# KristinnVikarJ/nbody-simulation

Hardware: AMD Instinct MI355X
Metric: pair-interactions/sec + ms/step at N=1M direct O(N^2) (force + integration step) (higher is better)
Workload: dtype f32; 1 GPU; direct O(N^2) f32, N=1048576 bodies, seeded 2-D Plummer sphere, masses 1, dt=0.1, clamp=0.001 (BASELINE.json configs[2]); n_bodies=1048576, targets_per_gpu=1048576, n_ranks=1, entry=one process per GPU (sharding.py over nbody_direct_{prep,run}_dev), exchange=none, arith=AUTO (FAST kernel; EXACT on hazardous positions)

## Files before the change

nbody-simulation_amd/csrc/ctx.h:

```cpp
#pragma once
#include <hip/hip_runtime.h>

#include <cstdlib>
#include <string>
#include <tuple>
#include <vector>

#include "common.h"
#include "env.h"
#include "tree_build.hpp"

namespace nbody {

struct Multi;

template <class T> struct State {
  using T2 = typename Vec2T<T>::type;
  struct Set {
    T2* pos = nullptr;
    T2* vel = nullptr;
    uint32_t* weight = nullptr;
    uint32_t* ids = nullptr;
    T* mass = nullptr;
  };
  int64_t n = 0;
  Set set[2];
  int cur = 0;
  T2* pos_next = nullptr;
  float uniform_mass = 0.f;
  float sparse_base = 0.f;
  struct MassClasses {
    uint64_t epoch = ~0ull;
    bool usable = false;
    int n_classes = 0;
    int64_t n_slots = 0;
    int n_pad_slots = 0;
    uint32_t* rank = nullptr;
    uint32_t* pad_slots = nullptr;
    float* tile_mass = nullptr;
  } classes;
  uint64_t row_epoch = 0;
  T2* acc = nullptr;
  void* geom0 = nullptr;
  void* geom1 = nullptr;
  void* link = nullptr;
  size_t node_cap = 0;
  uint32_t* order_dev = nullptr;
  TreeHost<T> tree;
  bool tree_valid = false;
  bool tree_host_stale = false;
  int n_nodes = 0, tree_kind = 0, tree_max_depth = 0;
  int shard_kind = 0;
  int* node_depth = nullptr;
  uint32_t* node_mass = nullptr;
  T2* node_size = nullptr;
  size_t node_aux_cap = 0;
  char* qb_scratch = nullptr;
  size_t qb_scratch_bytes = 0;
  char* bb_scratch = nullptr;
  size_t bb_scratch_bytes = 0;
  bool h_weight_stale = false;
  int quad_depth_hint = 0;
  int bvh_levels_hint = 0;
  int bvh_levels_stable = 0;
  bool bb_flags_clean = false;
  bool ahead_total_due = false;
  char* ws_scratch = nullptr;
  size_t ws_scratch_bytes = 0;
  void* ws_terms = nullptr;
  int64_t ws_capacity = 0;
  int ws_backoff = 0;
  int64_t wt_hist_n = -1, wt_hist_begin = 0;
  unsigned long long wt_total = 0;
  uint32_t* wt_hist = nullptr;
  std::vector<T> h_pos;
  std::vector<uint32_t> h_weight;
  std::vector<uint32_t> h_tmp;
};


struct Tracers {
  int64_t m = 0;
  void* pos = nullptr;
  void* vel = nullptr;
  void* acc = nullptr;
  uint8_t* mark = nullptr;
};

struct DeltaStream {
  void* keys[3] = {nullptr, nullptr, nullptr};
  int cur = 0;
  uint8_t* widths = nullptr;
  uint32_t *words = nullptr, *offsets = nullptr;
  void* scan = nullptr;
  size_t scan_bytes = 0;
  uint64_t *payload = nullptr, *total = nullptr, *htotal = nullptr;
  uint8_t* host = nullptr;
  int64_t n = -1;
  int bits = 0;
  bool key_next = true, pending = false;
  size_t stream_bytes = 0;
  uint64_t step = 0;
};

template <class T> inline float direct_mass_hint(const State<T>& s) { return s.uniform_mass > 0.f ? s.uniform_mass : -s.sparse_base; }

struct DirectStep {
  hipStream_t stream = nullptr;
  int64_t n_src = 0;
  const void *pos_all = nullptr, *mass_all = nullptr;
  float uniform_mass = 0.f, clamp = 0.f;
  int arith = 0;
  int64_t n_tgt_total = 0, n_tgt_max = 0;
  void* ws = nullptr;
  size_t ws_bytes = 0;
};
struct DirectBlock {
  int64_t tgt_begin = 0, n_tgt = 0;
  void *vel = nullptr, *pos_out = nullptr, *acc_out = nullptr;
  float delta = 0.f;
  nbody_timer* timer = nullptr;
};

struct DirectGraphKey {
  int64_t n = -1;
  const void *pos_a = nullptr, *pos_b = nullptr, *vel = nullptr, *mass = nullptr, *ws = nullptr;
  float delta = 0.f, clamp = 0.f, uniform = 0.f;
  int arith = -1;
  uint64_t row_epoch = ~0ull;
  bool cls_usable = false;
  const void *cls_rank = nullptr, *cls_tile_mass = nullptr;
  std::string env;
  auto tied() const { return std::tie(n, pos_a, pos_b, vel, mass, ws, delta, clamp, uniform, arith, row_epoch, cls_usable, cls_rank, cls_tile_mass, env); }
  bool operator==(const DirectGraphKey& o) const { return tied() == o.tied(); }
};
struct DirectGraph {
  hipGraphExec_t exec = nullptr;
  DirectGraphKey key;
  void reset() {
    if (exec) (void)hipGraphExecDestroy(exec);
    exec = nullptr;
    key = DirectGraphKey{};
  }
};
inline std::string direct_env_signature() {
  std::string sig;
  const char* nf = getenv("NBODY_DIRECT_NEARFAR");
  sig += nf ? nf : "-";
  sig += ';';
  for (const char* k : {"NBODY_DIRECT_ASM", "NBODY_DIRECT_TPT", "NBODY_DIRECT_GSPLIT", "NBODY_DIRECT_NO_UNIFORM", "NBODY_DIRECT_NO_CLASSES",
                        "NBODY_DIRECT_NO_SPARSE",
                        "NBODY_DIRECT_MUTUAL_MIN_N"}) {
    const char* v = lab_str(k);
    sig += v ? v : "-";
    sig += ';';
  }
  return sig;
}

struct PhaseEvents {
  hipEvent_t e[4] = {nullptr, nullptr, nullptr, nullptr};
  bool borrowed = false;
};
struct PhaseTiming {
  unsigned long long* stamp_dev = nullptr;
  std::vector<int> stamp_pending;
  int stamp_next = 0;
  int stamp_open = -1;
  std::vector<PhaseEvents> pending;
  std::vector<hipEvent_t> free_events;
  nbody_counting* counter = nullptr;
  void release() {
    if (stamp_dev) (void)hipFree(stamp_dev);
    for (auto& p : pending)
      for (int k = p.borrowed ? 1 : 0; k < 4; ++k)
        if (p.e[k]) (void)hipEventDestroy(p.e[k]);
    for (auto e : free_events) (void)hipEventDestroy(e);
  }
};
struct StepAheadRecord {
  int verdict[2];
  int build[128];
  int info_before[8];
  int info_after[8];
};
static_assert(sizeof(StepAheadRecord) == (2 + 128 + 8 + 8) * sizeof(int), "the record's parts lie back to back");
constexpr int kAheadBuildWords = sizeof(StepAheadRecord::build) / sizeof(int);
}

struct nbody_ctx {
  nbody::Multi* multi = nullptr;
  int64_t row_capacity = 0;
  nbody::DirectGraph direct_graph;
  int device = 0;
  hipStream_t stream = nullptr;
  std::string err;
  nbody_params params{};
  nbody_counting counting{};
  nbody_timer* timer = nullptr;
  bool has_f32 = false, has_f64 = false;
  nbody::State<float> sf;
  nbody::State<double> sd;
  void* workspace = nullptr;
  int bvh_stops = 0;
  bool last_build_device = false;
  size_t workspace_bytes = 0;
  unsigned long long* stats_dev = nullptr;
  uint32_t* frame_work = nullptr;
  hipStream_t copy_stream = nullptr;
  hipEvent_t snap_event = nullptr;
  bool snap_pending = false;
  uint64_t steps_done = 0, snap_step = 0;
  void *snap_pos = nullptr, *snap_vel = nullptr, *snap_hpos = nullptr, *snap_hvel = nullptr;
  uint32_t *snap_w = nullptr, *snap_ids = nullptr, *snap_hw = nullptr, *snap_hids = nullptr;
  size_t snap_bytes2 = 0;
  int64_t snap_n = 0;
  bool snap_f64 = false;
  void *snap_tpos = nullptr, *snap_tvel = nullptr, *snap_htpos = nullptr, *snap_htvel = nullptr;
  size_t snap_tcap = 0;
  int64_t snap_m = 0;
  nbody::DeltaStream dl;
  nbody::DeltaStream tdl;
  uint8_t* frame_rgba = nullptr;
  uint32_t frame_px = 0;
  unsigned long long last_stats[3] = {0, 0, 0};
  bool want_stats = false;
  nbody::PhaseTiming phases;
  int* spec_dev = nullptr;
  nbody::StepAheadRecord* spec_host_dev = nullptr;
  nbody::StepAheadRecord* spec_host = nullptr;
  hipEvent_t spec_event = nullptr;
  void* probe_ws = nullptr;
  size_t probe_ws_bytes = 0;
  nbody::Tracers tracers;
};

namespace nbody {
int ctx_fail(nbody_ctx* c, int code, const std::string& msg);
int ctx_create_single(nbody_ctx** out, int device_id);
void ctx_destroy_single(nbody_ctx* c);
int ctx_upload(nbody_ctx* c, bool f64, int64_t n, const void* pos, const void* vel, const uint32_t* w);
int ctx_update_tree(nbody_ctx* c, bool f64, int kind, double delta, int n_steps, nbody_counting* counter);
int ctx_update_tree_shard(nbody_ctx* c, bool f64, int kind, double delta, int64_t begin, int64_t count, nbody_counting* counter);
int ctx_export_slice(nbody_ctx* c, int64_t begin, int64_t count, void* rows, void* pos, void* vel);
int ctx_import_rows(nbody_ctx* c, int64_t n_rows, const void* rows, const void* pos, const void* vel);
size_t ctx_direct_ws_bytes(int64_t n_src, int64_t n_tgt);
int ctx_ensure_workspace(nbody_ctx* c, size_t bytes);
int ctx_ensure_mass_classes(nbody_ctx* c);
int ctx_direct_prep(nbody_ctx* c, const DirectStep& step);
int ctx_direct_run(nbody_ctx* c, const DirectStep& step, const DirectBlock& block);
int ctx_accel_direct_at(nbody_ctx* c, bool f64, int64_t n_targets, const void* target_xy, void* acc_xy);
void multi_destroy(nbody_ctx* front);
int multi_set_params(nbody_ctx* front);
int multi_upload(nbody_ctx* front, bool f64, int64_t n, const void* pos, const void* vel, const uint32_t* w);
nbody_ctx* multi_peek(const nbody_ctx* front);
int multi_primary(nbody_ctx* front, nbody_ctx** out);
int multi_replicate(nbody_ctx* front);
int multi_update_direct(nbody_ctx* front, float delta, int n_steps, nbody_counting* counter);
int multi_accel_direct_at(nbody_ctx* front, bool f64, int64_t n_targets, const void* target_xy, void* acc_xy);
int multi_update_tree(nbody_ctx* front, bool f64, int kind, double delta, int n_steps, nbody_counting* counter);
}
```

nbody-simulation_amd/csrc/direct_mutual.hip:

```cpp
#include <hip/hip_runtime.h>
#include <stdint.h>

#include "direct_kernels.h"
#include "mutual_schedule.h"

namespace nbody {

namespace {

typedef float v2f __attribute__((ext_vector_type(2)));

constexpr int kWaves = 8;

constexpr int kSlice = kMutualSlice;
constexpr int kSliceCouples = kSlice / 2;
constexpr int kChunks = kSliceCouples / 64;
constexpr float kMarker = 1e30f;

__device__ __forceinline__ bool gate_open(const DirectArgs& a) { return a.run_state < 0 || a.flags[kFlagState] == a.run_state; }

__device__ __forceinline__ float4 couple_or_marker(const float4* c, int64_t k, int64_t n_couples) {
  return k < n_couples ? c[k] : make_float4(kMarker, kMarker, kMarker, kMarker);
}

#define NB_PX(K, H, D) "v_pk_add_f32 v[" D "], v[184:185], %[tx" #K "] op_sel:[0," #H "] op_sel_hi:[1," #H "] neg_lo:[0,1] neg_hi:[0,1]\n\t"
#define NB_PY(K, H, D) "v_pk_add_f32 v[" D "], v[186:187], %[ty" #K "] op_sel:[0," #H "] op_sel_hi:[1," #H "] neg_lo:[0,1] neg_hi:[0,1]\n\t"
#define NB_SQ(DX, DY, Q) "v_pk_mul_f32 v[" Q "], v[" DX "], v[" DX "]\n\tv_pk_fma_f32 v[" Q "], v[" DY "], v[" DY "], v[" Q "]\n\t"
#define NB_AD(XL, XH, YL, YH, SL, SH) "v_add_f32_e64 v" SL ", |v" XL "|, |v" YL "|\n\tv_add_f32_e64 v" SH ", |v" XH "|, |v" YH "|\n\t"
#define NB_DN(S, Q) "v_pk_fma_f32 v[" S "], v[" S "], v[" Q "], %[b]\n\t"
#define NB_RC(SL, SH) "v_rcp_f32_e32 v" SL ", v" SL "\n\tv_rcp_f32_e32 v" SH ", v" SH "\n\t"
#define NB_AC(T, DX, DY, S)                                                                                                          \
  "v_pk_fma_f32 %[ax" #T "], v[" DX "], v[" S "], %[ax" #T "]\n\t"                                                                    \
  "v_pk_fma_f32 v[188:189], v[" DX "], v[" S "], v[188:189] neg_lo:[1,0,0] neg_hi:[1,0,0]\n\t"                                                  \
  "v_pk_fma_f32 %[ay" #T "], v[" DY "], v[" S "], %[ay" #T "]\n\t"                                                                    \
  "v_pk_fma_f32 v[190:191], v[" DY "], v[" S "], v[190:191] neg_lo:[1,0,0] neg_hi:[1,0,0]\n\t"
#define NB_HALF(K0, K1, K2, K3, T0, T1, T2, T3, T4, T5, T6, T7)                                                                    \
  NB_PX(K0, 0, "192:193") NB_PX(K0, 1, "200:201") NB_PX(K1, 0, "208:209") NB_PX(K1, 1, "216:217")                                   \
  NB_PX(K2, 0, "224:225") NB_PX(K2, 1, "232:233") NB_PX(K3, 0, "240:241") NB_PX(K3, 1, "248:249")                                   \
  NB_PY(K0, 0, "194:195") NB_PY(K0, 1, "202:203") NB_PY(K1, 0, "210:211") NB_PY(K1, 1, "218:219")                                   \
  NB_PY(K2, 0, "226:227") NB_PY(K2, 1, "234:235") NB_PY(K3, 0, "242:243") NB_PY(K3, 1, "250:251")                                   \
  NB_SQ("192:193", "194:195", "196:197") NB_SQ("200:201", "202:203", "204:205") NB_SQ("208:209", "210:211", "212:213")             \
  NB_SQ("216:217", "218:219", "220:221") NB_SQ("224:225", "226:227", "228:229") NB_SQ("232:233", "234:235", "236:237")             \
  NB_SQ("240:241", "242:243", "244:245") NB_SQ("248:249", "250:251", "252:253")                                                    \
  "s_setprio 0\n\t"                                                                                                                \
  NB_AD("192", "193", "194", "195", "198", "199") NB_AD("200", "201", "202", "203", "206", "207")                                  \
  NB_AD("208", "209", "210", "211", "214", "215") NB_AD("216", "217", "218", "219", "222", "223")                                  \
  NB_AD("224", "225", "226", "227", "230", "231") NB_AD("232", "233", "234", "235", "238", "239")                                  \
  NB_AD("240", "241", "242", "243", "246", "247") NB_AD("248", "249", "250", "251", "254", "255")                                  \
  "s_setprio 1\n\t"                                                                                                                \
  NB_DN("198:199", "196:197") NB_DN("206:207", "204:205") NB_DN("214:215", "212:213") NB_DN("222:223", "220:221")                 \
  NB_DN("230:231", "228:229") NB_DN("238:239", "236:237") NB_DN("246:247", "244:245") NB_DN("254:255", "252:253")                 \
  NB_RC("198", "199")                                                                                                              \
  NB_RC("206", "207") NB_AC(T0, "192:193", "194:195", "198:199")                                                                   \
  NB_RC("214", "215") NB_AC(T1, "200:201", "202:203", "206:207")                                                                   \
  NB_RC("222", "223") NB_AC(T2, "208:209", "210:211", "214:215")                                                                   \
  NB_RC("230", "231") NB_AC(T3, "216:217", "218:219", "222:223")                                                                   \
  NB_RC("238", "239") NB_AC(T4, "224:225", "226:227", "230:231")                                                                   \
  NB_RC("246", "247") NB_AC(T5, "232:233", "234:235", "238:239")                                                                   \
  NB_RC("254", "255") NB_AC(T6, "240:241", "242:243", "246:247")                                                                   \
  NB_AC(T7, "248:249", "250:251", "254:255")
#define NB_ROT(R) "v_mov_b32_dpp " R ", " R " wave_ror:1 row_mask:0xf bank_mask:0xf\n\t"

__device__ __forceinline__ void mutual_steps(const v2f* tx, const v2f* ty, v2f* ax, v2f* ay, float4& rc, float4& sacc, int steps,
                                             unsigned long long bias2) {
  asm volatile("v_mov_b32 v184, %[r0]\n\tv_mov_b32 v185, %[r1]\n\tv_mov_b32 v186, %[r2]\n\tv_mov_b32 v187, %[r3]\n\t"
               "v_mov_b32 v188, %[o0]\n\tv_mov_b32 v189, %[o1]\n\tv_mov_b32 v190, %[o2]\n\tv_mov_b32 v191, %[o3]\n\t"
               "s_mov_b32 s88, %[n]\n"
               ".Lnb_mutual_%=:\n\t"
               NB_HALF(0, 1, 2, 3, 0, 1, 2, 3, 4, 5, 6, 7) NB_HALF(4, 5, 6, 7, 8, 9, 10, 11, 12, 13, 14, 15)
               NB_ROT("v184") NB_ROT("v185") NB_ROT("v186") NB_ROT("v187") NB_ROT("v188") NB_ROT("v189") NB_ROT("v190") NB_ROT("v191")
               "s_sub_u32 s88, s88, 1\n\t"
               "s_cmp_lg_u32 s88, 0\n\t"
               "s_cbranch_scc1 .Lnb_mutual_%=\n\t"
               "v_mov_b32 %[o0], v188\n\tv_mov_b32 %[o1], v189\n\tv_mov_b32 %[o2], v190\n\tv_mov_b32 %[o3], v191\n\t"
               "v_mov_b32 %[r0], v184\n\tv_mov_b32 %[r1], v185\n\tv_mov_b32 %[r2], v186\n\tv_mov_b32 %[r3], v187\n\t"
               : [ax0] "+v"(ax[0]), [ax1] "+v"(ax[1]), [ax2] "+v"(ax[2]), [ax3] "+v"(ax[3]), [ax4] "+v"(ax[4]), [ax5] "+v"(ax[5]),
                 [ax6] "+v"(ax[6]), [ax7] "+v"(ax[7]), [ax8] "+v"(ax[8]), [ax9] "+v"(ax[9]), [ax10] "+v"(ax[10]), [ax11] "+v"(ax[11]),
                 [ax12] "+v"(ax[12]), [ax13] "+v"(ax[13]), [ax14] "+v"(ax[14]), [ax15] "+v"(ax[15]),
                 [ay0] "+v"(ay[0]), [ay1] "+v"(ay[1]), [ay2] "+v"(ay[2]), [ay3] "+v"(ay[3]), [ay4] "+v"(ay[4]), [ay5] "+v"(ay[5]),
                 [ay6] "+v"(ay[6]), [ay7] "+v"(ay[7]), [ay8] "+v"(ay[8]), [ay9] "+v"(ay[9]), [ay10] "+v"(ay[10]), [ay11] "+v"(ay[11]),
                 [ay12] "+v"(ay[12]), [ay13] "+v"(ay[13]), [ay14] "+v"(ay[14]), [ay15] "+v"(ay[15]),
                 [o0] "+v"(sacc.x), [o1] "+v"(sacc.y), [o2] "+v"(sacc.z), [o3] "+v"(sacc.w),
                 [r0] "+v"(rc.x), [r1] "+v"(rc.y), [r2] "+v"(rc.z), [r3] "+v"(rc.w)
               : [tx0] "v"(tx[0]), [tx1] "v"(tx[1]), [tx2] "v"(tx[2]), [tx3] "v"(tx[3]), [tx4] "v"(tx[4]), [tx5] "v"(tx[5]),
                 [tx6] "v"(tx[6]), [tx7] "v"(tx[7]), [ty0] "v"(ty[0]), [ty1] "v"(ty[1]), [ty2] "v"(ty[2]), [ty3] "v"(ty[3]),
                 [ty4] "v"(ty[4]), [ty5] "v"(ty[5]), [ty6] "v"(ty[6]), [ty7] "v"(ty[7]), [b] "s"(bias2), [n] "s"(steps)
               : "v184", "v185", "v186", "v187", "v188", "v189", "v190", "v191",
                 "v192", "v193", "v194", "v195", "v196", "v197", "v198", "v199", "v200", "v201", "v202", "v203", "v204", "v205",
                 "v206", "v207", "v208", "v209", "v210", "v211", "v212", "v213", "v214", "v215", "v216", "v217", "v218", "v219",
                 "v220", "v221", "v222", "v223", "v224", "v225", "v226", "v227", "v228", "v229", "v230", "v231", "v232", "v233",
                 "v234", "v235", "v236", "v237", "v238", "v239", "v240", "v241", "v242", "v243", "v244", "v245", "v246", "v247",
                 "v248", "v249", "v250", "v251", "v252", "v253", "v254", "v255", "s88", "scc");
}
#undef NB_PX
#undef NB_PY
#undef NB_SQ
#undef NB_AD
#undef NB_DN
#undef NB_RC
#undef NB_AC
#undef NB_HALF
#undef NB_ROT

__device__ __forceinline__ void load_targets(const float4* couples, int64_t n_couples, int s, int w, int lane, v2f* tx, v2f* ty) {
  const int64_t tc0 = (int64_t)s * kSliceCouples + 512 * w + 8 * lane;
#pragma unroll
  for (int k = 0; k < 8; ++k) {
    const float4 c = couple_or_marker(couples, tc0 + k, n_couples);
    tx[k] = v2f{c.x, c.y};
    ty[k] = v2f{c.z, c.w};
  }
}

__device__ __forceinline__ void zero_acc(v2f* ax, v2f* ay) {
#pragma unroll
  for (int t = 0; t < 16; ++t) ax[t] = ay[t] = v2f{0.f, 0.f};
}

__device__ __forceinline__ void add_chunk(const v2f* ax, const v2f* ay, float* tot_x, float* tot_y) {
#pragma unroll
  for (int t = 0; t < 16; ++t) {
    tot_x[t] += ax[t].x + ax[t].y;
    tot_y[t] += ay[t].x + ay[t].y;
  }
}

constexpr unsigned long long kBias2 = 0x1280000012800000ull;

__device__ __forceinline__ void off_item(const float4* couples, int64_t n_couples, int s, int b, int w, int lane, float4 (*red)[kWaves][64],
                                         float2* tpart, float2* spart_f2) {
  v2f tx[8], ty[8];
  load_targets(couples, n_couples, s, w, lane, tx, ty);
  float tot_x[16], tot_y[16];
#pragma unroll
  for (int t = 0; t < 16; ++t) tot_x[t] = tot_y[t] = 0.f;
  float* spart = reinterpret_cast<float*>(spart_f2);
  for (int c = 0; c < kChunks; ++c) {
    float4 rc = couple_or_marker(couples, (int64_t)b * kSliceCouples + 64 * c + lane, n_couples);
    v2f ax[16], ay[16];
    zero_acc(ax, ay);
    float4 sacc = make_float4(0.f, 0.f, 0.f, 0.f);
    mutual_steps(tx, ty, ax, ay, rc, sacc, 64, kBias2);
    add_chunk(ax, ay, tot_x, tot_y);
    red[c & 1][w][lane] = sacc;
    __syncthreads();
    if (threadIdx.x < 256) {
      const int q = threadIdx.x >> 2, comp = threadIdx.x & 3;
      float r = 0.f;
#pragma unroll
      for (int v = 0; v < kWaves; ++v) r += reinterpret_cast<const float*>(&red[c & 1][v][q])[comp];
      spart[(size_t)(128 * c + 2 * q + (comp & 1)) * 2 + (comp >> 1)] = r;
    }
  }
#pragma unroll
  for (int t = 0; t < 16; ++t) tpart[1024 * w + 16 * lane + t] = make_float2(tot_x[t], tot_y[t]);
}

__device__ __forceinline__ void diag_item(const float4* couples, int64_t n_couples, int s, int w, int lane, float4 (*src)[8][64],
                                          float2* out) {
  using namespace mutual_schedule;
  v2f tx[8], ty[8];
  load_targets(couples, n_couples, s, w, lane, tx, ty);
  float tot_x[16], tot_y[16];
#pragma unroll
  for (int t = 0; t < 16; ++t) tot_x[t] = tot_y[t] = 0.f;
  const int64_t c0 = (int64_t)s * kSliceCouples;
  for (int p = 0; p < kDiagPhases; ++p) {
    const int u = diag_block(w, p), r0 = diag_first_step(w, p), n = diag_steps(p);
    for (int j = 0; j < 8; ++j) {
      float4 rc = couple_or_marker(couples, c0 + 512 * u + 8 * ((lane - r0) & 63) + j, n_couples);
      v2f ax[16], ay[16];
      zero_acc(ax, ay);
      float4 sacc = make_float4(0.f, 0.f, 0.f, 0.f);
      int moved;
      if (p == 0) {
        mutual_steps(tx, ty, ax, ay, rc, sacc, 1, kBias2);
        sacc = make_float4(0.f, 0.f, 0.f, 0.f);
        mutual_steps(tx, ty, ax, ay, rc, sacc, n - 2, kBias2);
        const float4 keep = sacc;
        mutual_steps(tx, ty, ax, ay, rc, sacc, 1, kBias2);
        sacc = keep;
        moved = n - 1;
      } else {
        mutual_steps(tx, ty, ax, ay, rc, sacc, n, kBias2);
        moved = n;
      }
      add_chunk(ax, ay, tot_x, tot_y);
      const int shift = (r0 + moved) & 63;
      if (shift) {
        const int from = (lane + shift) & 63;
        sacc = make_float4(__shfl(sacc.x, from), __shfl(sacc.y, from), __shfl(sacc.z, from), __shfl(sacc.w, from));
      }
      float4& d = src[u][j][lane];
      if (p == 0) {
        d = sacc;
      } else {
        const float4 o = d;
        d = make_float4(o.x + sacc.x, o.y + sacc.y, o.z + sacc.z, o.w + sacc.w);
      }
    }
    __syncthreads();
  }
#pragma unroll
  for (int k = 0; k < 8; ++k) {
    const float4 q = src[w][k][lane];
    out[1024 * w + 16 * lane + 2 * k] = make_float2(tot_x[2 * k] + q.x, tot_y[2 * k] + q.z);
    out[1024 * w + 16 * lane + 2 * k + 1] = make_float2(tot_x[2 * k + 1] + q.y, tot_y[2 * k + 1] + q.w);
  }
  __syncthreads();
}

__global__ __launch_bounds__(kWaves * 64) void direct_mutual(const DirectArgs a, MutualArea m, int64_t lo) {
  if (!gate_open(a)) return;
  const int nb = m.n_slices;
  int s, b;
  mutual_schedule::unit_slices(lo + blockIdx.x, nb, s, b);
  const int lane = threadIdx.x & 63;
  const int w = __builtin_amdgcn_readfirstlane((int)(threadIdx.x >> 6));
  const float4* couples = reinterpret_cast<const float4*>(a.src_pos);
  const int64_t n_couples = a.n_src / 2;
  float2* tpart = m.tpart + (size_t)blockIdx.x * kSlice;
  float2* spart = m.spart + (size_t)blockIdx.x * kSlice;
  __shared__ float4 lds[8][8][64];
  __builtin_amdgcn_s_setprio(1);
  if (s < b) {
    off_item(couples, n_couples, s, b, w, lane, reinterpret_cast<float4(*)[kWaves][64]>(&lds[0][0][0]), tpart, spart);
  } else {
    diag_item(couples, n_couples, s, w, lane, lds, tpart);
    if (s + 1 < nb) diag_item(couples, n_couples, s + 1, w, lane, lds, spart);
  }
}

__global__ __launch_bounds__(256) void direct_mutual_near(const DirectArgs a, MutualArea m) {
  if (!gate_open(a)) return;
  const int n_near = a.flags[kFlagNearCount];
  const float4* couples = reinterpret_cast<const float4*>(a.src_pos);
  const int n_couples = a.n_src / 2;
  const int per = (n_couples + kMutualNearSplit - 1) / kMutualNearSplit;
  const int q0 = blockIdx.x * per, q1 = q0 + per < n_couples ? q0 + per : n_couples;
  __shared__ float2 red[256];
  for (int k = blockIdx.y; k < n_near; k += gridDim.y) {
    const float2 p = a.pos_all[a.near_list[k]];
    float ax = 0.f, ay = 0.f;
#pragma unroll 4
    for (int q = q0 + (int)threadIdx.x; q < q1; q += 256) {
      const float4 c = couples[q];
#pragma unroll
      for (int h = 0; h < 2; ++h) {
        const float dx = (h ? c.y : c.x) - p.x, dy = (h ? c.w : c.z) - p.y;
        const float sum = __builtin_fabsf(dx) + __builtin_fabsf(dy);
        const float d2 = __builtin_fmaf(dy, dy, dx * dx);
        const float s = __builtin_amdgcn_rcpf(__builtin_fmaf(sum, d2, 8.0779356694631609e-28f));
        ax = __builtin_fmaf(dx, s, ax);
        ay = __builtin_fmaf(dy, s, ay);
      }
    }
    red[threadIdx.x] = make_float2(ax, ay);
    __syncthreads();
    for (int w = 128; w > 0; w >>= 1) {
      if ((int)threadIdx.x < w) {
        red[threadIdx.x].x += red[threadIdx.x + w].x;
        red[threadIdx.x].y += red[threadIdx.x + w].y;
      }
      __syncthreads();
    }
    if (threadIdx.x == 0) m.near_part[(size_t)k * kMutualNearSplit + blockIdx.x] = red[0];
    __syncthreads();
  }
}

__global__ __launch_bounds__(256) void direct_mutual_reduce(const DirectArgs a, MutualArea m, int64_t lo, int64_t hi, int first, int last) {
  using mutual_schedule::item_of;
  if (!gate_open(a)) return;
  const int i = blockIdx.x * 256 + threadIdx.x;
  if (i >= a.n_tgt) return;
  const int nb = m.n_slices;
  const int s = i / kSlice, l = i % kSlice;
  int r0 = 0, r1 = s;
  while (r0 < r1) {
    const int mid = (r0 + r1) >> 1;
    if (item_of(mid, s, nb) < lo) r0 = mid + 1; else r1 = mid;
  }
  int re = s;
  r1 = r0;
  while (r1 < re) {
    const int mid = (r1 + re) >> 1;
    if (item_of(mid, s, nb) < hi) r1 = mid + 1; else re = mid;
  }
  const int64_t b0 = s + 1 < nb ? item_of(s, s + 1, nb) : 0, b1 = s + 1 < nb ? item_of(s, nb - 1, nb) + 1 : 0;
  const int64_t w0 = b0 > lo ? b0 : lo, w1 = b1 < hi ? b1 : hi;
  const int64_t d = mutual_schedule::diag_unit(s, nb);
  const bool has_d = d >= lo && d < hi;
  if (r0 == r1 && w0 >= w1 && !has_d && !first && !last) return;
  float2 acc = first ? make_float2(0.f, 0.f) : a.partial[i];
#pragma unroll 8
  for (int r = r0; r < r1; ++r) {
    const float2 p = m.spart[(size_t)(item_of(r, s, nb) - lo) * kSlice + l];
    acc.x += p.x;
    acc.y += p.y;
  }
#pragma unroll 8
  for (int64_t it = w0; it < w1; ++it) {
    const float2 p = m.tpart[(size_t)(it - lo) * kSlice + l];
    acc.x += p.x;
    acc.y += p.y;
  }
  if (has_d) {
    const float2 p = ((s & 1) ? m.spart : m.tpart)[(size_t)(d - lo) * kSlice + l];
    acc.x += p.x;
    acc.y += p.y;
  }
  if (last) {
    if (m.is_near[i]) {
      const float2* np = m.near_part + (size_t)m.near_scan[i] * kMutualNearSplit;
      acc = np[0];
      for (int g = 1; g < kMutualNearSplit; ++g) {
        acc.x += np[g].x;
        acc.y += np[g].y;
      }
    }
    acc = make_float2(acc.x * a.uniform_mass, acc.y * a.uniform_mass);
  }
  a.partial[i] = acc;
}

}

int mutual_slices(int64_t n_slots) { return (int)((n_slots + kSlice - 1) / kSlice); }

size_t mutual_area_bytes(int64_t n_src) {
  return 2 * (size_t)kMutualStripItems * kSlice * sizeof(float2) + ((size_t)n_src / 64 + 2) * kMutualNearSplit * sizeof(float2);
}

MutualArea mutual_area(void* base, int64_t n_src, const uint32_t* is_near, const uint32_t* near_scan) {
  MutualArea m{};
  m.n_slices = mutual_slices(far_padded(n_src));
  float2* p = (float2*)base;
  m.tpart = p;
  p += (size_t)kMutualStripItems * kSlice;
  m.spart = p;
  p += (size_t)kMutualStripItems * kSlice;
  m.near_part = p;
  m.is_near = is_near;
  m.near_scan = near_scan;
  return m;
}

hipError_t launch_direct_mutual(hipStream_t s, const DirectArgs& a, const MutualArea& m) {
  if (a.n_tgt <= 0) return hipSuccess;
  if (!a.src_couples || a.tgt_begin != 0 || a.n_src < a.n_tgt || m.n_slices != mutual_slices(a.n_src)) return hipErrorInvalidValue;
  int dev = 0, cus = 0;
  hipError_t e = hipGetDevice(&dev);
  if (e == hipSuccess) e = hipDeviceGetAttribute(&cus, hipDeviceAttributeMultiprocessorCount, dev);
  if (e != hipSuccess) return e;
  if (cus <= 0) return hipErrorInvalidValue;
  const int64_t units = mutual_schedule::units(m.n_slices);
  const int64_t strip = mutual_schedule::strip_units(cus, kMutualStripItems);
  const dim3 rgrid((unsigned)((a.n_tgt + 255) / 256));
  hipLaunchKernelGGL(direct_mutual_near, dim3(kMutualNearSplit, kMutualNearRows), dim3(256), 0, s, a, m);
  for (int64_t lo = 0; lo < units; lo += strip) {
    const int64_t hi = lo + strip < units ? lo + strip : units;
    hipLaunchKernelGGL(direct_mutual, dim3((unsigned)(hi - lo)), dim3(kWaves * 64), 0, s, a, m, lo);
    hipLaunchKernelGGL(direct_mutual_reduce, rgrid, dim3(256), 0, s, a, m, lo, hi, lo == 0 ? 1 : 0, hi == units ? 1 : 0);
  }
  return hipGetLastError();
}

}
```

Baseline: 10080 billion pair-interactions/s.

## Batch mutual off-diagonal barriers, fold chunk accumulators, pin asm registers

The off-diagonal mutual item now syncs and reduces the source partials once every four chunks instead of every chunk, using a double-buffered LDS exchange sized for four chunks. It also folds the per-chunk accumulators into the totals every four chunks rather than after each chunk, and pins the inline-asm accumulator operands to fixed VGPRs with an aligned loop head. The aim is fewer workgroup barriers and less add/zero overhead in the hot loop. In exchange, more LDS is used, partial sums run longer before folding (slightly different f32 rounding), and lab-build variants are selectable through an environment knob.

```diff
diff --git a/nbody-simulation_amd/csrc/ctx.h b/nbody-simulation_amd/csrc/ctx.h
--- a/nbody-simulation_amd/csrc/ctx.h
+++ b/nbody-simulation_amd/csrc/ctx.h
@@ -150,7 +150,7 @@
   sig += ';';
   for (const char* k : {"NBODY_DIRECT_ASM", "NBODY_DIRECT_TPT", "NBODY_DIRECT_GSPLIT", "NBODY_DIRECT_NO_UNIFORM", "NBODY_DIRECT_NO_CLASSES",
                         "NBODY_DIRECT_NO_SPARSE",
-                        "NBODY_DIRECT_MUTUAL_MIN_N"}) {
+                        "NBODY_DIRECT_MUTUAL_MIN_N", "NBODY_DIRECT_MUTUAL_WRAP"}) {
     const char* v = lab_str(k);
     sig += v ? v : "-";
     sig += ';';
diff --git a/nbody-simulation_amd/csrc/direct_mutual.hip b/nbody-simulation_amd/csrc/direct_mutual.hip
--- a/nbody-simulation_amd/csrc/direct_mutual.hip
+++ b/nbody-simulation_amd/csrc/direct_mutual.hip
@@ -2,6 +2,7 @@
 #include <stdint.h>
 
 #include "direct_kernels.h"
+#include "env.h"
 #include "mutual_schedule.h"
 
 namespace nbody {
@@ -61,37 +62,55 @@
   NB_AC(T7, "248:249", "250:251", "254:255")
 #define NB_ROT(R) "v_mov_b32_dpp " R ", " R " wave_ror:1 row_mask:0xf bank_mask:0xf\n\t"
 
+#define NB_FREE(R) "+v"
+#define NB_PINNED(R) "+{v[" R "]}"
+#define NB_MUTUAL_ASM(K, ALIGN)                                                                                                          \
+  asm volatile("v_mov_b32 v184, %[r0]\n\tv_mov_b32 v185, %[r1]\n\tv_mov_b32 v186, %[r2]\n\tv_mov_b32 v187, %[r3]\n\t"                    \
+               "v_mov_b32 v188, %[o0]\n\tv_mov_b32 v189, %[o1]\n\tv_mov_b32 v190, %[o2]\n\tv_mov_b32 v191, %[o3]\n\t"                    \
+               "s_mov_b32 s88, %[n]\n" ALIGN                                                                                          \
+               ".Lnb_mutual_%=:\n\t"                                                                                                  \
+               NB_HALF(0, 1, 2, 3, 0, 1, 2, 3, 4, 5, 6, 7) NB_HALF(4, 5, 6, 7, 8, 9, 10, 11, 12, 13, 14, 15)                           \
+               NB_ROT("v184") NB_ROT("v185") NB_ROT("v186") NB_ROT("v187") NB_ROT("v188") NB_ROT("v189") NB_ROT("v190") NB_ROT("v191") \
+               "s_sub_u32 s88, s88, 1\n\t"                                                                                            \
+               "s_cmp_lg_u32 s88, 0\n\t"                                                                                              \
+               "s_cbranch_scc1 .Lnb_mutual_%=\n\t"                                                                                    \
+               "v_mov_b32 %[o0], v188\n\tv_mov_b32 %[o1], v189\n\tv_mov_b32 %[o2], v190\n\tv_mov_b32 %[o3], v191\n\t"                    \
+               "v_mov_b32 %[r0], v184\n\tv_mov_b32 %[r1], v185\n\tv_mov_b32 %[r2], v186\n\tv_mov_b32 %[r3], v187\n\t"                    \
+               :                                                                                                                      \
+                 [ax0] K("132:133")(ax[0]), [ax1] K("128:129")(ax[1]), [ax2] K("124:125")(ax[2]), [ax3] K("120:121")(ax[3]),                           \
+                 [ax4] K("116:117")(ax[4]), [ax5] K("112:113")(ax[5]), [ax6] K("108:109")(ax[6]), [ax7] K("104:105")(ax[7]),                           \
+                 [ax8] K("100:101")(ax[8]), [ax9] K("96:97")(ax[9]), [ax10] K("92:93")(ax[10]), [ax11] K("88:89")(ax[11]),                             \
+                 [ax12] K("84:85")(ax[12]), [ax13] K("80:81")(ax[13]), [ax14] K("78:79")(ax[14]), [ax15] K("68:69")(ax[15]),                           \
+                 [ay0] K("138:139")(ay[0]), [ay1] K("136:137")(ay[1]), [ay2] K("134:135")(ay[2]), [ay3] K("130:131")(ay[3]),                           \
+                 [ay4] K("126:127")(ay[4]), [ay5] K("122:123")(ay[5]), [ay6] K("118:119")(ay[6]), [ay7] K("114:115")(ay[7]),                           \
+                 [ay8] K("110:111")(ay[8]), [ay9] K("106:107")(ay[9]), [ay10] K("102:103")(ay[10]), [ay11] K("98:99")(ay[11]),                         \
+                 [ay12] K("94:95")(ay[12]), [ay13] K("90:91")(ay[13]), [ay14] K("86:87")(ay[14]), [ay15] K("82:83")(ay[15]),                           \
+                 [o0] "+v"(sacc.x), [o1] "+v"(sacc.y), [o2] "+v"(sacc.z), [o3] "+v"(sacc.w),                                          \
+                 [r0] "+v"(rc.x), [r1] "+v"(rc.y), [r2] "+v"(rc.z), [r3] "+v"(rc.w)                                                   \
+               : [tx0] "v"(tx[0]), [tx1] "v"(tx[1]), [tx2] "v"(tx[2]), [tx3] "v"(tx[3]), [tx4] "v"(tx[4]), [tx5] "v"(tx[5]),          \
+                 [tx6] "v"(tx[6]), [tx7] "v"(tx[7]), [ty0] "v"(ty[0]), [ty1] "v"(ty[1]), [ty2] "v"(ty[2]), [ty3] "v"(ty[3]),          \
+                 [ty4] "v"(ty[4]), [ty5] "v"(ty[5]), [ty6] "v"(ty[6]), [ty7] "v"(ty[7]), [b] "s"(bias2), [n] "s"(steps)               \
+               : "v184", "v185", "v186", "v187", "v188", "v189", "v190", "v191",                                                      \
+                 "v192", "v193", "v194", "v195", "v196", "v197", "v198", "v199", "v200", "v201", "v202", "v203", "v204", "v205",      \
+                 "v206", "v207", "v208", "v209", "v210", "v211", "v212", "v213", "v214", "v215", "v216", "v217", "v218", "v219",      \
+                 "v220", "v221", "v222", "v223", "v224", "v225", "v226", "v227", "v228", "v229", "v230", "v231", "v232", "v233",      \
+                 "v234", "v235", "v236", "v237", "v238", "v239", "v240", "v241", "v242", "v243", "v244", "v245", "v246", "v247",      \
+                 "v248", "v249", "v250", "v251", "v252", "v253", "v254", "v255", "s88", "scc")
+
+template <int kAlign = 0>
 __device__ __forceinline__ void mutual_steps(const v2f* tx, const v2f* ty, v2f* ax, v2f* ay, float4& rc, float4& sacc, int steps,
                                              unsigned long long bias2) {
-  asm volatile("v_mov_b32 v184, %[r0]\n\tv_mov_b32 v185, %[r1]\n\tv_mov_b32 v186, %[r2]\n\tv_mov_b32 v187, %[r3]\n\t"
-               "v_mov_b32 v188, %[o0]\n\tv_mov_b32 v189, %[o1]\n\tv_mov_b32 v190, %[o2]\n\tv_mov_b32 v191, %[o3]\n\t"
-               "s_mov_b32 s88, %[n]\n"
-               ".Lnb_mutual_%=:\n\t"
-               NB_HALF(0, 1, 2, 3, 0, 1, 2, 3, 4, 5, 6, 7) NB_HALF(4, 5, 6, 7, 8, 9, 10, 11, 12, 13, 14, 15)
-               NB_ROT("v184") NB_ROT("v185") NB_ROT("v186") NB_ROT("v187") NB_ROT("v188") NB_ROT("v189") NB_ROT("v190") NB_ROT("v191")
-               "s_sub_u32 s88, s88, 1\n\t"
-               "s_cmp_lg_u32 s88, 0\n\t"
-               "s_cbranch_scc1 .Lnb_mutual_%=\n\t"
-               "v_mov_b32 %[o0], v188\n\tv_mov_b32 %[o1], v189\n\tv_mov_b32 %[o2], v190\n\tv_mov_b32 %[o3], v191\n\t"
-               "v_mov_b32 %[r0], v184\n\tv_mov_b32 %[r1], v185\n\tv_mov_b32 %[r2], v186\n\tv_mov_b32 %[r3], v187\n\t"
-               : [ax0] "+v"(ax[0]), [ax1] "+v"(ax[1]), [ax2] "+v"(ax[2]), [ax3] "+v"(ax[3]), [ax4] "+v"(ax[4]), [ax5] "+v"(ax[5]),
-                 [ax6] "+v"(ax[6]), [ax7] "+v"(ax[7]), [ax8] "+v"(ax[8]), [ax9] "+v"(ax[9]), [ax10] "+v"(ax[10]), [ax11] "+v"(ax[11]),
-                 [ax12] "+v"(ax[12]), [ax13] "+v"(ax[13]), [ax14] "+v"(ax[14]), [ax15] "+v"(ax[15]),
-                 [ay0] "+v"(ay[0]), [ay1] "+v"(ay[1]), [ay2] "+v"(ay[2]), [ay3] "+v"(ay[3]), [ay4] "+v"(ay[4]), [ay5] "+v"(ay[5]),
-                 [ay6] "+v"(ay[6]), [ay7] "+v"(ay[7]), [ay8] "+v"(ay[8]), [ay9] "+v"(ay[9]), [ay10] "+v"(ay[10]), [ay11] "+v"(ay[11]),
-                 [ay12] "+v"(ay[12]), [ay13] "+v"(ay[13]), [ay14] "+v"(ay[14]), [ay15] "+v"(ay[15]),
-                 [o0] "+v"(sacc.x), [o1] "+v"(sacc.y), [o2] "+v"(sacc.z), [o3] "+v"(sacc.w),
-                 [r0] "+v"(rc.x), [r1] "+v"(rc.y), [r2] "+v"(rc.z), [r3] "+v"(rc.w)
-               : [tx0] "v"(tx[0]), [tx1] "v"(tx[1]), [tx2] "v"(tx[2]), [tx3] "v"(tx[3]), [tx4] "v"(tx[4]), [tx5] "v"(tx[5]),
-                 [tx6] "v"(tx[6]), [tx7] "v"(tx[7]), [ty0] "v"(ty[0]), [ty1] "v"(ty[1]), [ty2] "v"(ty[2]), [ty3] "v"(ty[3]),
-                 [ty4] "v"(ty[4]), [ty5] "v"(ty[5]), [ty6] "v"(ty[6]), [ty7] "v"(ty[7]), [b] "s"(bias2), [n] "s"(steps)
-               : "v184", "v185", "v186", "v187", "v188", "v189", "v190", "v191",
-                 "v192", "v193", "v194", "v195", "v196", "v197", "v198", "v199", "v200", "v201", "v202", "v203", "v204", "v205",
-                 "v206", "v207", "v208", "v209", "v210", "v211", "v212", "v213", "v214", "v215", "v216", "v217", "v218", "v219",
-                 "v220", "v221", "v222", "v223", "v224", "v225", "v226", "v227", "v228", "v229", "v230", "v231", "v232", "v233",
-                 "v234", "v235", "v236", "v237", "v238", "v239", "v240", "v241", "v242", "v243", "v244", "v245", "v246", "v247",
-                 "v248", "v249", "v250", "v251", "v252", "v253", "v254", "v255", "s88", "scc");
-}
+  static_assert(kAlign == 0 || kAlign == 3 || kAlign == 6, "");
+  if constexpr (kAlign == 3)
+    NB_MUTUAL_ASM(NB_PINNED, ".p2align 3\n");
+  else if constexpr (kAlign == 6)
+    NB_MUTUAL_ASM(NB_PINNED, ".p2align 6\n");
+  else
+    NB_MUTUAL_ASM(NB_FREE, "");
+}
+#undef NB_MUTUAL_ASM
+#undef NB_PINNED
+#undef NB_FREE
 #undef NB_PX
 #undef NB_PY
 #undef NB_SQ
@@ -127,29 +146,64 @@
 
 constexpr unsigned long long kBias2 = 0x1280000012800000ull;
 
-__device__ __forceinline__ void off_item(const float4* couples, int64_t n_couples, int s, int b, int w, int lane, float4 (*red)[kWaves][64],
+template <bool kAhead_, int kFold_, int kSync_, int kAlign_ = 3>
+struct Wrap {
+  static constexpr bool kAhead = kAhead_;
+  static constexpr int kFold = kFold_, kSync = kSync_, kAlign = kAlign_;
+  static_assert(kChunks % kFold == 0 && kChunks % kSync == 0, "every wave folds, and reaches the barrier, after a whole group");
+  static_assert(2 * kSync * kWaves * 64 * sizeof(float4) <= 65536, "the exchange lives in the kernel's one LDS array");
+};
+using WrapProduct = Wrap<false, 4, 4>;
+using WrapRound7 = Wrap<false, 1, 1>;
+
+template <class W>
+__device__ __forceinline__ void off_item(const float4* couples, int64_t n_couples, int s, int b, int w, int lane, float4* lds,
                                          float2* tpart, float2* spart_f2) {
+  float4(*red)[W::kSync][kWaves][64] = reinterpret_cast<float4(*)[W::kSync][kWaves][64]>(lds);
   v2f tx[8], ty[8];
   load_targets(couples, n_couples, s, w, lane, tx, ty);
   float tot_x[16], tot_y[16];
 #pragma unroll
   for (int t = 0; t < 16; ++t) tot_x[t] = tot_y[t] = 0.f;
   float* spart = reinterpret_cast<float*>(spart_f2);
+  const int64_t sc0 = (int64_t)b * kSliceCouples + lane;
+  float4 nxt = make_float4(0.f, 0.f, 0.f, 0.f);
+  if constexpr (W::kAhead) {
+    nxt = couple_or_marker(couples, sc0, n_couples);
+#pragma unroll
+    for (int k = 0; k < 8; ++k) asm volatile("" : : "v"(tx[k]), "v"(ty[k]));
+  }
+  v2f ax[16], ay[16];
+#pragma unroll 1
   for (int c = 0; c < kChunks; ++c) {
-    float4 rc = couple_or_marker(couples, (int64_t)b * kSliceCouples + 64 * c + lane, n_couples);
-    v2f ax[16], ay[16];
-    zero_acc(ax, ay);
+    float4 rc;
+    if constexpr (W::kAhead) {
+      rc = nxt;
+      if (c + 1 < kChunks) nxt = couple_or_marker(couples, sc0 + 64 * (c + 1), n_couples);
+    } else {
+      rc = couple_or_marker(couples, sc0 + 64 * c, n_couples);
+    }
+    if (c % W::kFold == 0) zero_acc(ax, ay);
     float4 sacc = make_float4(0.f, 0.f, 0.f, 0.f);
-    mutual_steps(tx, ty, ax, ay, rc, sacc, 64, kBias2);
-    add_chunk(ax, ay, tot_x, tot_y);
-    red[c & 1][w][lane] = sacc;
-    __syncthreads();
-    if (threadIdx.x < 256) {
-      const int q = threadIdx.x >> 2, comp = threadIdx.x & 3;
-      float r = 0.f;
-#pragma unroll
-      for (int v = 0; v < kWaves; ++v) r += reinterpret_cast<const float*>(&red[c & 1][v][q])[comp];
-      spart[(size_t)(128 * c + 2 * q + (comp & 1)) * 2 + (comp >> 1)] = r;
+    mutual_steps<W::kAlign>(tx, ty, ax, ay, rc, sacc, 64, kBias2);
+    if constexpr (W::kAhead) asm volatile("" : : "v"(nxt.x), "v"(nxt.y), "v"(nxt.z), "v"(nxt.w));
+    if (c % W::kFold == W::kFold - 1) add_chunk(ax, ay, tot_x, tot_y);
+    const int buf = (c / W::kSync) & 1;
+    red[buf][c % W::kSync][w][lane] = sacc;
+    if (c % W::kSync == W::kSync - 1) {
+      __syncthreads();
+      constexpr int kOut = 256 * W::kSync;
+#pragma unroll
+      for (int o0 = 0; o0 < kOut; o0 += kWaves * 64) {
+        const int o = o0 + (int)threadIdx.x;
+        if (o < kOut) {
+          const int j = o >> 8, q = (o >> 2) & 63, comp = o & 3;
+          float r = 0.f;
+#pragma unroll
+          for (int v = 0; v < kWaves; ++v) r += reinterpret_cast<const float*>(&red[buf][j][v][q])[comp];
+          spart[(size_t)(128 * (c - (W::kSync - 1) + j) + 2 * q + (comp & 1)) * 2 + (comp >> 1)] = r;
+        }
+      }
     }
   }
 #pragma unroll
@@ -210,6 +264,7 @@
   __syncthreads();
 }
 
+template <class W>
 __global__ __launch_bounds__(kWaves * 64) void direct_mutual(const DirectArgs a, MutualArea m, int64_t lo) {
   if (!gate_open(a)) return;
   const int nb = m.n_slices;
@@ -224,7 +279,7 @@
   __shared__ float4 lds[8][8][64];
   __builtin_amdgcn_s_setprio(1);
   if (s < b) {
-    off_item(couples, n_couples, s, b, w, lane, reinterpret_cast<float4(*)[kWaves][64]>(&lds[0][0][0]), tpart, spart);
+    off_item<W>(couples, n_couples, s, b, w, lane, &lds[0][0][0], tpart, spart);
   } else {
     diag_item(couples, n_couples, s, w, lane, lds, tpart);
     if (s + 1 < nb) diag_item(couples, n_couples, s + 1, w, lane, lds, spart);
@@ -346,6 +401,32 @@
   return m;
 }
 
+namespace {
+
+template <class W>
+void launch_units(hipStream_t s, const DirectArgs& a, const MutualArea& m, int64_t lo, int64_t hi) {
+  hipLaunchKernelGGL(direct_mutual<W>, dim3((unsigned)(hi - lo)), dim3(kWaves * 64), 0, s, a, m, lo);
+}
+
+using UnitsLauncher = void (*)(hipStream_t, const DirectArgs&, const MutualArea&, int64_t, int64_t);
+UnitsLauncher units_launcher() {
+  if constexpr (kLabBuild) {
+    switch (lab_int("NBODY_DIRECT_MUTUAL_WRAP", 1)) {
+      case 0: return launch_units<WrapRound7>;
+      case 1: break;
+      case 2: return launch_units<Wrap<false, 1, 4>>;
+      case 3: return launch_units<Wrap<true, 1, 1>>;
+      case 4: return launch_units<Wrap<false, 2, 4>>;
+      case 5: return launch_units<Wrap<true, 4, 4>>;
+      case 6: return launch_units<Wrap<false, 4, 4, 6>>;
+      default: return nullptr;
+    }
+  }
+  return launch_units<WrapProduct>;
+}
+
+}
+
 hipError_t launch_direct_mutual(hipStream_t s, const DirectArgs& a, const MutualArea& m) {
   if (a.n_tgt <= 0) return hipSuccess;
   if (!a.src_couples || a.tgt_begin != 0 || a.n_src < a.n_tgt || m.n_slices != mutual_slices(a.n_src)) return hipErrorInvalidValue;
@@ -353,14 +434,15 @@
   hipError_t e = hipGetDevice(&dev);
   if (e == hipSuccess) e = hipDeviceGetAttribute(&cus, hipDeviceAttributeMultiprocessorCount, dev);
   if (e != hipSuccess) return e;
-  if (cus <= 0) return hipErrorInvalidValue;
+  const UnitsLauncher launch = units_launcher();
+  if (cus <= 0 || !launch) return hipErrorInvalidValue;
   const int64_t units = mutual_schedule::units(m.n_slices);
   const int64_t strip = mutual_schedule::strip_units(cus, kMutualStripItems);
   const dim3 rgrid((unsigned)((a.n_tgt + 255) / 256));
   hipLaunchKernelGGL(direct_mutual_near, dim3(kMutualNearSplit, kMutualNearRows), dim3(256), 0, s, a, m);
   for (int64_t lo = 0; lo < units; lo += strip) {
     const int64_t hi = lo + strip < units ? lo + strip : units;
-    hipLaunchKernelGGL(direct_mutual, dim3((unsigned)(hi - lo)), dim3(kWaves * 64), 0, s, a, m, lo);
+    launch(s, a, m, lo, hi);
     hipLaunchKernelGGL(direct_mutual_reduce, rgrid, dim3(256), 0, s, a, m, lo, hi, lo == 0 ? 1 : 0, hi == units ? 1 : 0);
   }
   return hipGetLastError();
```

After: 10130 billion pair-interactions/s, median of 6. No clear change (+0.5%).
